# marcobellagente93/scaling

Hardware: AMD Instinct MI355X
Metric: tokens/sec (whole node) Llama-2-7B-shape bf16, TP×PP×DP on 1/2/4/8 MI355X (higher is better)
Workload: dtype bf16

## Files before the change

### csrc/bindings.cpp

```cpp
#include <torch/extension.h>
#include <ATen/hip/HIPContext.h>
#include <c10/core/DeviceGuard.h>

#include <atomic>
#include <cmath>
#include <cstring>
#include <string>
#include <vector>
#include "kernels/launch.h"

void register_rehearsal(pybind11::module& m);
void register_blaslt(pybind11::module& m);

namespace {

hipStream_t cur_stream() { return at::hip::getCurrentHIPStream().stream(); }

int dt(const at::Tensor& t) {
    switch (t.scalar_type()) {
        case at::kFloat: return DT_F32;
        case at::kBFloat16: return DT_BF16;
        case at::kHalf: return DT_F16;
        default: TORCH_CHECK(false, "scaling_amd: unsupported dtype ", t.scalar_type());
    }
// ... 632 lines not shown
        TORCH_CHECK(q.scalar_type() == at::kBFloat16, "flash_attn: FP8 k / v need bfloat16 queries (an e4m3 code times its scale is exact in bfloat16, not in float16)");
        TORCH_CHECK(v.size(0) == k.size(0), "flash_attn: k and v must hold the same number of rows");
        for (const at::Tensor* s : {&*k_scale, &*v_scale})
            TORCH_CHECK(s->is_cuda() && s->scalar_type() == at::kFloat && s->dim() == 2 && s->size(0) == k.size(1) &&
                            s->size(1) == k.size(0) && s->stride(1) == 1 && s->stride(0) == k_scale->stride(0),
                        "flash_attn: k_scale / v_scale must be float32 GPU tensors [kv heads, key rows] with unit last stride");
    } else {
        check_qkv(k, "k"); check_qkv(v, "v");
        TORCH_CHECK(k.scalar_type() == q.scalar_type() && v.scalar_type() == q.scalar_type(), "flash_attn: q/k/v dtypes differ");
    }
    TORCH_CHECK(p_drop >= 0.0 && p_drop < 1.0, "flash_attn: dropout probability must be in [0, 1)");
    const int64_t D = q.size(2);
    TORCH_CHECK(D == 32 || D == 64 || D == 128, "flash_attn: head dim must be 32, 64 or 128");
    TORCH_CHECK(k.size(2) == D && v.size(2) == D && k.size(1) == v.size(1) && q.size(1) % k.size(1) == 0, "flash_attn: shapes");
    TORCH_CHECK(cu_q.scalar_type() == at::kInt && cu_k.scalar_type() == at::kInt && cu_q.numel() == cu_k.numel(), "flash_attn: cu_seqlens int32");
    const at::DeviceGuard g(q.device());
    const int64_t T = q.size(0), H = q.size(1);
    auto o = at::empty({T, H, D}, q.options());
    auto lse = at::empty({H, T}, q.options().dtype(at::kFloat));
    FwdArgs a{};
    a.q = (const uint16_t*)q.data_ptr(); a.k = (const uint16_t*)k.data_ptr(); a.v = (const uint16_t*)v.data_ptr();
    a.o = (uint16_t*)o.data_ptr(); a.lse = lse.data_ptr<float>();
    a.q_tok = q.stride(0); a.q_head = q.stride(1); a.k_tok = k.stride(0); a.k_head = k.stride(1);
    a.v_tok = v.stride(0); a.v_head = v.stride(1); a.o_tok = o.stride(0); a.o_head = o.stride(1); a.lse_stride = T;
    a.cu_q = cu_q.data_ptr<int>(); a.cu_k = cu_k.data_ptr<int>();
    a.nseg = (int)cu_q.numel() - 1; a.Hq = (int)H; a.Hkv = (int)k.size(1); a.causal = causal ? 1 : 0; a.window = (int)window;
    a.local_heads = local_heads < 0 ? (int)H : (int)local_heads;
    a.scale_log2 = (float)(scale * 1.4426950408889634);
    a.p_drop = (float)p_drop; a.rp_drop = (float)(1.0 / (1.0 - p_drop)); a.seed = (uint32_t)seed; a.drop_thr = drop_threshold(p_drop);
    const int64_t grp = H / k.size(1);
    if (k_range.has_value()) {
        TORCH_CHECK(k_range->is_cuda() && k_range->scalar_type() == at::kInt && k_range->is_contiguous() &&
                    k_range->dim() == 2 && k_range->size(0) == a.nseg && k_range->size(1) == 2,
                    "flash_attn: k_range must be a contiguous int32 GPU tensor [nseg, 2]");
        TORCH_CHECK(p_drop == 0.0 && max_q * grp <= 32,
                    "flash_attn: key ranges are supported by the decode kernel only (max_q * heads per kv head <= 32, "
                    "no dropout)");
        TORCH_CHECK(v.size(0) == k.size(0), "flash_attn: k and v must hold the same number of rows");
    }
    if (block_table.has_value()) {
        TORCH_CHECK(k_range.has_value(), "flash_attn: block_table needs k_range (start 0, length per segment)");
        TORCH_CHECK(page_size > 0 && page_size % 32 == 0, "flash_attn: page_size must be a positive multiple of 32");
        TORCH_CHECK(block_table->is_cuda() && block_table->scalar_type() == at::kInt && block_table->dim() == 2 &&
                    block_table->size(0) == a.nseg && block_table->size(1) >= 1 && block_table->stride(1) == 1,
                    "flash_attn: block_table must be an int32 GPU tensor [nseg, max_pages] with unit last stride");
        TORCH_CHECK(k.size(0) > 0 && k.size(0) % page_size == 0 && k.size(0) < (int64_t)1 << 31 &&
                    block_table->size(1) * page_size < (int64_t)1 << 31,
                    "flash_attn: with block_table, k / v must hold a whole number of pages (fewer than 2^31 rows)");
    }
    if (q8)
        TORCH_CHECK(p_drop == 0.0 && max_q * grp <= 32,
                    "flash_attn: FP8 k / v are supported by the decode kernel only (max_q * heads per kv head <= 32, "
                    "no dropout)");
    if (T > 0 && a.nseg > 0 && p_drop == 0.0 && max_q * grp <= 32) {
        DecArgs d{};
        d.q = a.q; d.k = a.k; d.v = a.v;
        d.q_tok = a.q_tok; d.q_head = a.q_head; d.k_tok = a.k_tok; d.k_head = a.k_head; d.v_tok = a.v_tok; d.v_head = a.v_head;
        d.cu_q = a.cu_q; d.cu_k = a.cu_k; d.nseg = a.nseg;
        if (q8) { d.k_scale = k_scale->data_ptr<float>(); d.v_scale = v_scale->data_ptr<float>(); d.s_head = k_scale->stride(0); }
        d.k_range = k_range.has_value() ? k_range->data_ptr<int>() : nullptr; d.k_rows = k.size(0); d.Hq = a.Hq; d.Hkv = a.Hkv; d.causal = a.causal;
        d.window = a.window; d.local_heads = a.local_heads; d.scale_log2 = a.scale_log2; d.Tq = T;
        if (block_table.has_value()) {
            d.block_table = block_table->data_ptr<int>(); d.bt_stride = block_table->stride(0); d.page = (int)page_size;
            d.num_pages = (int)(k.size(0) / page_size); d.max_pages = (int)block_table->size(1);
        }
        sa_launch::fa_decode_plan(max_k > 0 ? max_k : k.size(0), a.Hkv, a.nseg, d.split_keys, d.nsplit);
        auto part_o = at::empty({(int64_t)d.nsplit, T, H, D}, q.options().dtype(at::kFloat));
        auto part_ml = at::empty({(int64_t)d.nsplit, T, H, 2}, q.options().dtype(at::kFloat));
        d.part_o = part_o.data_ptr<float>(); d.part_ml = part_ml.data_ptr<float>();
        d.o = a.o; d.o_tok = a.o_tok; d.o_head = a.o_head; d.lse = a.lse; d.lse_stride = a.lse_stride;
        sa_launch::fa_decode(d, (int)D, q.scalar_type() == at::kHalf, cur_stream());
        return {o, lse};
    }
    if (T > 0 && a.nseg > 0) sa_launch::fa_fwd(a, (int)D, (int)max_q, q.scalar_type() == at::kHalf, cur_stream());
    return {o, lse};
}
std::vector<at::Tensor> fa_bwd(const at::Tensor& dout, const at::Tensor& q, const at::Tensor& k, const at::Tensor& v,
                               const at::Tensor& o, const at::Tensor& lse, const at::Tensor& cu_q, const at::Tensor& cu_k,
                               int64_t max_q, int64_t max_k, double scale, bool causal, int64_t window,
                               const c10::optional<at::Tensor>& dq_out, const c10::optional<at::Tensor>& dk_out,
                               const c10::optional<at::Tensor>& dv_out, double p_drop, int64_t seed, int64_t local_heads,
                               const c10::optional<at::Tensor>& rope_cos, const c10::optional<at::Tensor>& rope_sin,
                               const c10::optional<at::Tensor>& rope_pos, int64_t rope_dim, int64_t rope_seq,
                               bool rope_interleaved) {
    check_qkv(q, "q"); check_qkv(k, "k"); check_qkv(v, "v"); check_qkv(o, "o");
    TORCH_CHECK(k.scalar_type() == q.scalar_type() && v.scalar_type() == q.scalar_type() && o.scalar_type() == q.scalar_type() &&
                dout.scalar_type() == q.scalar_type(), "fa_bwd: dtypes differ");
    auto dO = dout.contiguous();
    check_qkv(dO, "dout");
    const int64_t D = q.size(2), T = q.size(0), H = q.size(1), Tk = k.size(0), Hk = k.size(1);
    const at::DeviceGuard g(q.device());
    auto take = [](const c10::optional<at::Tensor>& t, const at::Tensor& like, const char* n) {
        if (!t.has_value()) return at::empty(like.sizes(), like.options());
        TORCH_CHECK(t->sizes() == like.sizes() && t->scalar_type() == like.scalar_type(), "fa_bwd: ", n, " shape/dtype");
        check_qkv(*t, n);
        return *t;
    };
    auto dq = take(dq_out, q, "dq_out");
    auto dk = take(dk_out, k, "dk_out");
    auto dv = take(dv_out, v, "dv_out");
    auto delta = at::empty({H, T}, q.options().dtype(at::kFloat));
    auto lse2 = at::empty({H, T}, q.options().dtype(at::kFloat));
    BwdArgs a{};
    a.q = (const uint16_t*)q.data_ptr(); a.k = (const uint16_t*)k.data_ptr(); a.v = (const uint16_t*)v.data_ptr();
    a.dO = (const uint16_t*)dO.data_ptr(); a.lse = lse.data_ptr<float>(); a.delta = delta.data_ptr<float>(); a.lse2 = lse2.data_ptr<float>();
    a.dq = (uint16_t*)dq.data_ptr(); a.dk = (uint16_t*)dk.data_ptr(); a.dv = (uint16_t*)dv.data_ptr();
    a.q_tok = q.stride(0); a.q_head = q.stride(1); a.k_tok = k.stride(0); a.k_head = k.stride(1);
    a.v_tok = v.stride(0); a.v_head = v.stride(1); a.do_tok = dO.stride(0); a.do_head = dO.stride(1);
    a.dq_tok = dq.stride(0); a.dq_head = dq.stride(1); a.dk_tok = dk.stride(0); a.dk_head = dk.stride(1);
    a.dv_tok = dv.stride(0); a.dv_head = dv.stride(1); a.lse_stride = T;
    a.cu_q = cu_q.data_ptr<int>(); a.cu_k = cu_k.data_ptr<int>();
    a.nseg = (int)cu_q.numel() - 1; a.Hq = (int)H; a.Hkv = (int)Hk; a.causal = causal ? 1 : 0; a.window = (int)window;
    a.local_heads = local_heads < 0 ? (int)H : (int)local_heads;
    a.scale = (float)scale; a.scale_log2 = (float)(scale * 1.4426950408889634);
    a.p_drop = (float)p_drop; a.rp_drop = (float)(1.0 / (1.0 - p_drop)); a.seed = (uint32_t)seed; a.drop_thr = drop_threshold(p_drop);
    a.hsplit = 1; a.Tk = (int)Tk;
    const int grp = (int)(H / Hk);
    const int64_t kblocks = (max_k + 127) / 128;
    if (causal || window >= 0)
        while (a.hsplit < grp && grp % (2 * a.hsplit) == 0 && Hk * a.hsplit * a.nseg * kblocks < 1024) a.hsplit *= 2;
    at::Tensor part;
    if (a.hsplit > 1) {
        part = at::empty({2, a.hsplit, Tk, Hk, D}, q.options().dtype(at::kFloat));
        a.dk_part = part[0].data_ptr<float>();
        a.dv_part = part[1].data_ptr<float>();
    }
    const bool rope = rope_cos.has_value();
    bool fold = false;
    if (rope) {
        TORCH_CHECK(rope_sin.has_value() && rope_cos->scalar_type() == at::kFloat && rope_sin->scalar_type() == at::kFloat &&
                    rope_cos->is_contiguous() && rope_sin->is_contiguous() && rope_cos->size(-1) == rope_dim / 2 &&
                    (!rope_pos.has_value() ||
                     (rope_pos->scalar_type() == at::kLong && rope_pos->numel() == T && rope_pos->is_contiguous() &&
                      rope_pos->device() == q.device())),
                    "fa_bwd: rope tables / positions (contiguous fp32 tables, contiguous int64 positions of [T])");
        fold = D >= 64 && (rope_interleaved ? rope_dim <= D && rope_dim % 8 == 0 : rope_dim == D) && a.hsplit == 1 &&
               Tk == T;
        if (fold) {
            a.rcos = rope_cos->data_ptr<float>(); a.rsin = rope_sin->data_ptr<float>();
            a.rpos = rope_pos.has_value() ? rope_pos->data_ptr<int64_t>() : nullptr;
            a.rrd = (int)rope_dim; a.rseq = (int)rope_seq; a.ril = rope_interleaved ? 1 : 0;
        }
    }
    if (T > 0 && a.nseg > 0)
        sa_launch::fa_bwd(a, (const uint16_t*)o.data_ptr(), o.stride(0), o.stride(1), T, (int)D, (int)max_q, (int)max_k,
                          q.scalar_type() == at::kHalf, cur_stream());
    if (rope && !fold) {
        const int64_t* pp = rope_pos.has_value() ? rope_pos->data_ptr<int64_t>() : nullptr;
        for (at::Tensor* t : {&dq, &dk}) {
            sa_launch::rope(dt(*t), rope_interleaved, t->data_ptr(), t->stride(0), t->stride(1), t->data_ptr(),
                            t->stride(0), t->stride(1), rope_cos->data_ptr<float>(), rope_sin->data_ptr<float>(), pp,
                            t->size(0), (int)t->size(1), (int)t->size(2), (int)rope_dim, (int)rope_seq, -1.f,
                            cur_stream());
        }
    }
    return {dq, dk, dv};
}
at::Tensor aligned16(const at::Tensor& t) {
    auto c = t.contiguous();
    return (reinterpret_cast<uintptr_t>(c.data_ptr()) % 16 == 0) ? c : c.clone();
}
std::tuple<const void*, int64_t, int64_t, int64_t> mask_view(const c10::optional<at::Tensor>& mask, const at::Tensor& x,
                                                             at::Tensor& keep) {
    if (!mask.has_value()) return {nullptr, 0, 0, 0};
    TORCH_CHECK(mask->scalar_type() == at::kBool, "masked_softmax: mask must be bool");
    auto m = mask->to(x.device()).expand(x.sizes());
    if (m.stride(3) != 1) m = m.contiguous();
    keep = m;
    return {m.data_ptr(), m.stride(0), m.stride(1), m.stride(2)};
}
at::Tensor masked_softmax_fwd(const at::Tensor& x_, const c10::optional<at::Tensor>& mask, double scale, double fill,
                              bool round_scaled) {
    TORCH_CHECK(x_.is_cuda() && x_.dim() == 4, "masked_softmax: x must be a [B, H, Sq, Sk] GPU tensor");
    const at::DeviceGuard g(x_.device());
    auto x = aligned16(x_);
    at::Tensor keep;
    auto [mp, mb, mh, mq] = mask_view(mask, x, keep);
    auto y = at::empty_like(x);
    const int64_t N = x.size(3), rows = x.numel() / std::max<int64_t>(N, 1);
    if (rows > 0 && N > 0)
        sa_launch::masked_softmax_fwd(dt(x), x.data_ptr(), mp, y.data_ptr(), rows, (int)N, (int)x.size(1), (int)x.size(2), mb, mh,
                                      mq, (float)scale, (float)fill, round_scaled, cur_stream());
    return y;
}
at::Tensor masked_softmax_bwd(const at::Tensor& dy_, const at::Tensor& y_, const c10::optional<at::Tensor>& mask, double scale) {
    TORCH_CHECK(y_.is_cuda() && y_.dim() == 4 && dy_.sizes() == y_.sizes() && dy_.scalar_type() == y_.scalar_type(),
                "masked_softmax_bwd: shapes");
    const at::DeviceGuard g(y_.device());
    auto y = aligned16(y_);
    auto dy = aligned16(dy_);
    at::Tensor keep;
    auto [mp, mb, mh, mq] = mask_view(mask, y, keep);
    auto dx = at::empty_like(y);
    const int64_t N = y.size(3), rows = y.numel() / std::max<int64_t>(N, 1);
    if (rows > 0 && N > 0)
        sa_launch::masked_softmax_bwd(dt(y), dy.data_ptr(), y.data_ptr(), mp, dx.data_ptr(), rows, (int)N, (int)y.size(1),
                                      (int)y.size(2), mb, mh, mq, (float)scale, cur_stream());
    return dx;
}
at::Tensor act_fwd(const at::Tensor& x_, int64_t kind) {
    TORCH_CHECK(x_.is_cuda(), "activation: GPU tensor expected");
    const at::DeviceGuard g(x_.device());
    auto x = aligned16(x_);
    auto y = at::empty_like(x);
    if (x.numel() > 0) sa_launch::act_fwd(dt(x), x.data_ptr(), y.data_ptr(), x.numel(), (int)kind, cur_stream());
    return y;
}
at::Tensor act_bwd(const at::Tensor& dy_, const at::Tensor& x_, int64_t kind) {
    TORCH_CHECK(x_.is_cuda() && dy_.sizes() == x_.sizes() && dy_.scalar_type() == x_.scalar_type(), "activation_bwd: shapes");
    const at::DeviceGuard g(x_.device());
    auto x = aligned16(x_);
    auto dy = aligned16(dy_);
    auto dx = at::empty_like(x);
    if (x.numel() > 0) sa_launch::act_bwd(dt(x), dy.data_ptr(), x.data_ptr(), dx.data_ptr(), x.numel(), (int)kind, cur_stream());
    return dx;
}
void spin_us(int64_t us) { sa_launch::spin(us, cur_stream()); }
int64_t gate_flags_alloc(int64_t n) {
    void* p = nullptr;
    const size_t bytes = (size_t)std::max<int64_t>(n, 1) * sizeof(uint32_t);
    TORCH_CHECK(hipHostMalloc(&p, bytes, hipHostMallocCoherent | hipHostMallocMapped) == hipSuccess, "gate: pinned memory");
    std::memset(p, 0, bytes);
    return (int64_t)(uintptr_t)p;
}
void gate_flag_write(int64_t base, int64_t idx, int64_t value) {
    std::atomic_thread_fence(std::memory_order_seq_cst);
    __atomic_store_n(reinterpret_cast<uint32_t*>((uintptr_t)base) + idx, (uint32_t)value, __ATOMIC_SEQ_CST);
}
int64_t gate_flag_read(int64_t base, int64_t idx) {
// ... 64 lines not shown
    m.def("sample_max_resident_vocab", []() { return sa_launch::sample_max_resident(); },
          "the largest vocabulary whose row the sampling kernel stages in LDS");
    m.doc() = "scaling_amd CDNA4 (gfx950) HIP kernels";
    register_rehearsal(m);
    register_blaslt(m);
    m.def("norm_fwd", &norm_fwd, "RMSNorm/LayerNorm forward (optional fused residual add)", py::arg("x"), py::arg("w"), py::arg("b"), py::arg("eps"), py::arg("layer"), py::arg("res") = py::none());
    m.def("norm_bwd", &norm_bwd, "RMSNorm/LayerNorm backward (optional fused residual-gradient add)", py::arg("dy"), py::arg("x"), py::arg("w"), py::arg("mean"), py::arg("rstd"), py::arg("layer"), py::arg("dadd") = py::none());
    m.def("swiglu_fwd", &swiglu_fwd, "SwiGLU forward");
    m.def("swiglu_bwd", &swiglu_bwd, "SwiGLU backward");
    m.def("ar_alloc", &ar_alloc, "one-shot all-reduce: allocate + IPC-export a registered buffer");
    m.def("ar_open", &ar_open, "one-shot all-reduce: map a peer's registered buffer");
    m.def("ar_close", &ar_close, "unmap a peer buffer");
    m.def("ar_free", &ar_free, "free an own registered buffer");
    m.def("ar_allreduce", &ar_allreduce, "one-shot all-reduce of x over the registered buffers (in place)",
          py::arg("x"), py::arg("bases"), py::arg("rank"), py::arg("slot_off"), py::arg("flag_off"), py::arg("epoch"),
          py::arg("signal"), py::arg("err"), py::arg("max_spins") = int64_t(1) << 26);
    m.def("transpose_ok", &transpose_ok, "whether transpose2d supports this tensor");
    m.def("transpose2d", &transpose2d, "x^T (contiguous) for 2-byte 2-D matrices");
    m.def("gemv_ok", &gemv_ok, "whether gemv supports these operands");
    m.def("gemv", &gemv, "y = x W^T (+ b) for at most 4 rows of x (decode-time linear layers)", py::arg("x"), py::arg("W"), py::arg("bias") = py::none());
    m.def("gemv_residual", &gemv_residual, "y = x W^T + res for at most 4 rows (decode MLP-out + residual)");
    m.def("gemv_swiglu", &gemv_swiglu, "y = silu(x Wg^T) * (x Wu^T) for W = [Wg; Wu], at most 4 rows (decode)");
    m.def("gemv_w8_ok", &gemv_w8_ok, "whether the FP8-weight GEMV supports these operands");
    m.def("gemv_w8", &gemv_w8, "y = x (scale * Q)^T (+ b) for at most 4 bf16 rows of x, Q e4m3fn codes, scale fp32 per row",
          py::arg("x"), py::arg("q"), py::arg("scale"), py::arg("bias") = py::none());
    m.def("gemv_w8_residual", &gemv_w8_residual, "gemv_w8 + res (decode down / o-projection + residual)");
    m.def("gemv_w8_swiglu", &gemv_w8_swiglu, "silu(x Wg^T) * (x Wu^T) over FP8 [Wg; Wu] with per-row scales (decode)");
    m.def("gemv_w8_norm_ok", &gemv_w8_norm_ok, "whether gemv_w8_norm supports these operands");
    m.def("gemv_w8_norm", &gemv_w8_norm, "(s, gemv_w8(rms_norm(s), Q, scale)) with s = x (+ add); epi 0 plain, 2 SwiGLU",
          py::arg("x"), py::arg("add"), py::arg("gamma"), py::arg("eps"), py::arg("q"), py::arg("scale"), py::arg("epi") = 0);
    m.def("gemv_norm_ok", &gemv_norm_ok, "whether gemv_norm supports these operands");
    m.def("gemv_norm_rope", &gemv_norm_rope, "graph decode: rms_norm + q/k/v GEMV + interleaved RoPE + K/V cache append "
          "in one launch; returns q or None");
    m.def("gemv_norm", &gemv_norm, "(s, gemv(rms_norm(s), W)) with s = x (+ add); epi 0 plain, 2 SwiGLU (decode)",
          py::arg("x"), py::arg("add"), py::arg("gamma"), py::arg("eps"), py::arg("W"), py::arg("epi") = 0);
    m.def("skinny_ok", &skinny_ok, "whether skinny supports these operands");
    m.def("skinny", &skinny, "y = x W^T (+ b) for at most 16 rows of x on the MFMA weight-streaming kernel (batched decode)",
          py::arg("x"), py::arg("W"), py::arg("bias") = py::none());
    m.def("skinny_residual", &skinny_residual, "y = x W^T + res for at most 16 rows (decode down / o-projection + residual)");
    m.def("skinny_swiglu", &skinny_swiglu, "y = silu(x Wg^T) * (x Wu^T) for W = [Wg; Wu], at most 16 rows (decode)");
    m.def("skinny_norm_ok", &skinny_norm_ok, "whether skinny_norm supports these operands");
    m.def("skinny_norm", &skinny_norm, "(s, skinny(rms_norm(s), W)) with s = x (+ add); epi 0 plain, 2 SwiGLU (decode)",
          py::arg("x"), py::arg("add"), py::arg("gamma"), py::arg("eps"), py::arg("W"), py::arg("epi") = 0);
    m.def("skinny_w8_ok", &skinny_w8_ok, "whether the FP8-weight skinny kernel supports these operands");
    m.def("skinny_w8", &skinny_w8, "y = x (scale * Q)^T (+ b) for at most 16 bf16 rows of x, Q e4m3fn codes, scale fp32 per row",
          py::arg("x"), py::arg("q"), py::arg("scale"), py::arg("bias") = py::none());
    m.def("skinny_w8_residual", &skinny_w8_residual, "skinny_w8 + res (decode down / o-projection + residual)");
    m.def("skinny_w8_swiglu", &skinny_w8_swiglu, "silu(x Wg^T) * (x Wu^T) over FP8 [Wg; Wu] with per-row scales (decode)");
    m.def("skinny_w8_norm_ok", &skinny_w8_norm_ok, "whether skinny_w8_norm supports these operands");
    m.def("skinny_w8_norm", &skinny_w8_norm, "(s, skinny_w8(rms_norm(s), Q, scale)) with s = x (+ add); epi 0 plain, 2 SwiGLU",
          py::arg("x"), py::arg("add"), py::arg("gamma"), py::arg("eps"), py::arg("q"), py::arg("scale"), py::arg("epi") = 0);
    m.def("gemm_tn_ok", &gemm_tn_ok, "whether gemm_tn supports these operands");
    m.def("gemm_tn", &gemm_tn, "C (+)= A^T B for k-major bf16 operands (weight-gradient GEMM)");
    m.def("rope", &rope, "rotary embedding (fwd / inverse), optional strided / in-place output", py::arg("x"), py::arg("cos"), py::arg("sin"), py::arg("pos"), py::arg("rot_dim"), py::arg("seq_len"), py::arg("interleaved"), py::arg("inverse"), py::arg("out") = py::none());
    m.def("rope_kv_append", &rope_kv_append, "graph decode: RoPE q, RoPE k into the K cache row, v into the V cache row (k_scale / v_scale: FP8 e4m3 cache)",
          py::arg("qkv"), py::arg("cos"), py::arg("sin"), py::arg("pos"), py::arg("nq"), py::arg("nkv"), py::arg("rot_dim"), py::arg("interleaved"),
          py::arg("kc"), py::arg("vc"), py::arg("err"), py::arg("k_scale") = py::none(), py::arg("v_scale") = py::none());
    m.def("rope_kv_append_batch", &rope_kv_append_batch, "batched graph decode: rope_kv_append for one token of each of B sequences, one launch",
          py::arg("qkv"), py::arg("cos"), py::arg("sin"), py::arg("pos"), py::arg("nq"), py::arg("nkv"), py::arg("rot_dim"), py::arg("interleaved"),
          py::arg("kc"), py::arg("vc"), py::arg("err"), py::arg("cap"), py::arg("k_scale") = py::none(), py::arg("v_scale") = py::none());
    m.def("rope_kv_append_paged", &rope_kv_append_paged, "paged batched decode: rope_kv_append_batch into the pages a block table names, one launch",
          py::arg("qkv"), py::arg("cos"), py::arg("sin"), py::arg("pos"), py::arg("nq"), py::arg("nkv"), py::arg("rot_dim"), py::arg("interleaved"),
          py::arg("kc"), py::arg("vc"), py::arg("err"), py::arg("block_table"), py::arg("page"), py::arg("k_scale") = py::none(), py::arg("v_scale") = py::none());
    m.def("xent_stats", &xent_stats, "cross-entropy row statistics");
    m.def("xent_bwd", &xent_bwd, "cross-entropy backward");
    m.def("embed_fwd", &embed_fwd, "vocab-parallel embedding forward");
    m.def("embed_bwd", &embed_bwd, "deterministic embedding backward", py::call_guard<py::gil_scoped_release>());
    m.def("adamw_", &adamw_, "fused AdamW on flat fp32 buffers");
    m.def("sumsq_", &sumsq_, "sum of squares + non-finite count");
    m.def("cast_scale_", &cast_scale_, "y = cast(x * scale)");
    m.def("masked_softmax_fwd", &masked_softmax_fwd, "softmax(masked_fill(x * scale, mask, fill)) over the last dim", py::arg("x"), py::arg("mask"), py::arg("scale"), py::arg("fill"), py::arg("round_scaled"));
    m.def("masked_softmax_bwd", &masked_softmax_bwd, "masked softmax backward", py::arg("dy"), py::arg("y"), py::arg("mask"), py::arg("scale"));
    m.def("act_fwd", &act_fwd, "activation forward (0 gelu, 1 silu, 2 gelu-tanh)");
    m.def("act_bwd", &act_bwd, "activation backward");
    m.def("spin_us", &spin_us, "debug: busy-wait kernel of ~us microseconds on the current stream");
    m.def("gate_flags_alloc", &gate_flags_alloc, "stream gates: n flag words (coherent pinned host memory)");
    m.def("gate_flag_write", &gate_flag_write, "stream gates: host store of a flag word (after a full fence)");
    m.def("gate_flag_read", &gate_flag_read, "stream gates: host load of a flag word");
    m.def("gate_stream_wait", &gate_stream_wait, "stream gates: the current stream waits until flag[idx] >= value");
    m.def("xgmi_emulate", &xgmi_emulate, "per-rank proxy: emulated collective (HBM traffic on nwg CUs, held to us)",
          py::arg("src"), py::arg("scratch"), py::arg("bytes"), py::arg("us"), py::arg("nwg") = 16);
    m.def("dropout_add", &dropout_add, "residual + dropout(x) with a hashed keep mask", py::arg("x"), py::arg("res"), py::arg("p"), py::arg("seed"));
    m.def("fa_fwd", &fa_fwd, "flash attention forward (bf16/fp16, optional attention dropout)", py::arg("q"), py::arg("k"), py::arg("v"), py::arg("cu_q"), py::arg("cu_k"), py::arg("max_q"), py::arg("scale"), py::arg("causal"), py::arg("window"), py::arg("p_drop") = 0.0, py::arg("seed") = 0, py::arg("local_heads") = -1, py::arg("max_k") = -1, py::arg("k_range") = py::none(), py::arg("k_scale") = py::none(), py::arg("v_scale") = py::none(), py::arg("block_table") = py::none(), py::arg("page_size") = 0);
    m.def("fa_bwd", &fa_bwd, "flash attention backward (optional strided dq/dk/dv outputs)", py::arg("dout"), py::arg("q"), py::arg("k"), py::arg("v"), py::arg("o"), py::arg("lse"), py::arg("cu_q"), py::arg("cu_k"), py::arg("max_q"), py::arg("max_k"), py::arg("scale"), py::arg("causal"), py::arg("window"), py::arg("dq_out") = py::none(), py::arg("dk_out") = py::none(), py::arg("dv_out") = py::none(), py::arg("p_drop") = 0.0, py::arg("seed") = 0, py::arg("local_heads") = -1, py::arg("rope_cos") = py::none(), py::arg("rope_sin") = py::none(), py::arg("rope_pos") = py::none(), py::arg("rope_dim") = 0, py::arg("rope_seq") = 1, py::arg("rope_interleaved") = false);
}
```

### csrc/kernels/flash_bwd.hip

```cpp
#include "flash_attn.h"
#include "launch.h"

using namespace sa;
using namespace sa::fa;

template <int D, typename E>
__global__ __launch_bounds__(256) void fa_bwd_dot_kernel(const E* __restrict__ o, int64_t o_tok, int64_t o_head,
                                                         const E* __restrict__ dO, int64_t d_tok, int64_t d_head,
                                                         float* __restrict__ delta, const float* __restrict__ lse,
                                                         float* __restrict__ lse2, int64_t T, int H) {
    constexpr int LPR = D / 8;
    const int64_t gid = (int64_t)blockIdx.x * blockDim.x + threadIdx.x;
    const int64_t row = gid / LPR;
    const int c = (int)(gid % LPR);
    float s = 0.f;
    const bool ok = row < T * H;
    int64_t t = 0;
    int hh = 0;
    if (ok) {
        t = row / H;
        hh = (int)(row % H);
        float a[8], b[8];
        V8<E>::ld(o + t * o_tok + hh * o_head + 8 * c, a);
        V8<E>::ld(dO + t * d_tok + hh * d_head + 8 * c, b);
#pragma unroll
        for (int j = 0; j < 8; ++j) s += a[j] * b[j];
    }
#pragma unroll
    for (int w = LPR / 2; w > 0; w >>= 1) s += __shfl_xor(s, w, 64);
    if (ok && c == 0) {
        delta[(int64_t)hh * T + t] = s;
        lse2[(int64_t)hh * T + t] = lse[(int64_t)hh * T + t] * 1.4426950408889634f;
    }
}

template <int D, bool F16>
__device__ __forceinline__ void store_grad_row(const BwdArgs& a, const f32x16 (&acc)[D / 32], float scale, int64_t tok,
                                               int h, u16* dst) {
    constexpr int NT = D / 32;
    auto rd = [&](int t, int g, float (&x)[4]) {
#pragma unroll
        for (int j = 0; j < 4; ++j) x[j] = t2f<F16>(f2t<F16>(acc[t][4 * g + j] * scale));
    };
    auto st = [&](int t, int g, const float (&x)[4]) {
        u16x4 w;
#pragma unroll
        for (int j = 0; j < 4; ++j) w[j] = f2t<F16>(x[j]);
        *reinterpret_cast<u16x4*>(dst + 32 * t + 8 * g + 4 * h) = w;
    };
    if (a.rcos == nullptr) {
#pragma unroll
        for (int t = 0; t < NT; ++t)
#pragma unroll
            for (int g = 0; g < 4; ++g) {
                float x[4];
                rd(t, g, x);
                st(t, g, x);
            }
        return;
    }
    const int64_t ps = a.rpos ? a.rpos[tok] : (tok % a.rseq);
    const float* cb = a.rcos + ps * (a.rrd / 2);
    const float* sb = a.rsin + ps * (a.rrd / 2);
    if constexpr (NT < 2) return;
    if (!a.ril) {
        constexpr int NH = NT / 2 > 0 ? NT / 2 : 1;
        f32x4 cv[NH][4], sv[NH][4];
#pragma unroll
        for (int t = 0; t < NT / 2; ++t)
#pragma unroll
            for (int g = 0; g < 4; ++g) {
                cv[t][g] = *reinterpret_cast<const f32x4*>(cb + 32 * t + 8 * g + 4 * h);
                sv[t][g] = *reinterpret_cast<const f32x4*>(sb + 32 * t + 8 * g + 4 * h);
            }
#pragma unroll
        for (int t = 0; t < NT / 2; ++t)
#pragma unroll
            for (int g = 0; g < 4; ++g) {
                float x[4], y[4];
                rd(t, g, x);
                rd(t + NT / 2, g, y);
#pragma unroll
                for (int j = 0; j < 4; ++j) {
                    float o0, o1;
                    rot_pair(x[j], y[j], cv[t][g][j], -sv[t][g][j], o0, o1);
                    x[j] = o0;
                    y[j] = o1;
                }
                st(t, g, x);
                st(t + NT / 2, g, y);
            }
        return;
    }
    const int hr = a.rrd / 2 - 2;
    float2 cv[NT][4], sv[NT][4];
#pragma unroll
    for (int t = 0; t < NT; ++t)
#pragma unroll
        for (int g = 0; g < 4; ++g) {
            const int p = min((32 * t + 8 * g + 4 * h) / 2, hr);
            cv[t][g] = *reinterpret_cast<const float2*>(cb + p);
            sv[t][g] = *reinterpret_cast<const float2*>(sb + p);
        }
#pragma unroll
    for (int t = 0; t < NT; ++t)
#pragma unroll
        for (int g = 0; g < 4; ++g) {
            const bool rot = 32 * t + 8 * g + 4 * h < a.rrd;
            float x[4];
// ... 182 lines not shown
        if (w + 2 < nwork) {
            issue(ig, iq, buf0);
            adv(ig, iq);
        }
        tile(buf1, cg, cq);
        adv(cg, cq);
        dma_barrier();
    }
    if (w < nwork) tile(buf0, cg, cq);

    if (mykey < Lk) {
        if (a.hsplit > 1) {
            const int64_t pix = (((int64_t)sub * a.Tk + k0s + mykey) * a.Hkv + hk) * D;
            float* kp = a.dk_part + pix;
            float* vp = a.dv_part + pix;
#pragma unroll
            for (int t = 0; t < NT; ++t)
#pragma unroll
                for (int g = 0; g < 4; ++g) {
                    f32x4 wk, wv;
#pragma unroll
                    for (int j = 0; j < 4; ++j) {
                        wk[j] = dk[t][4 * g + j] * a.scale;
                        wv[j] = dv[t][4 * g + j];
                    }
                    *reinterpret_cast<f32x4*>(kp + 32 * t + 8 * g + 4 * h) = wk;
                    *reinterpret_cast<f32x4*>(vp + 32 * t + 8 * g + 4 * h) = wv;
                }
        } else {
            u16* vp = a.dv + (int64_t)(k0s + mykey) * a.dv_tok + (int64_t)hk * a.dv_head;
#pragma unroll
            for (int t = 0; t < NT; ++t)
#pragma unroll
                for (int g = 0; g < 4; ++g) {
                    u16x4 wv;
#pragma unroll
                    for (int j = 0; j < 4; ++j) wv[j] = f2t<F16>(dv[t][4 * g + j]);
                    *reinterpret_cast<u16x4*>(vp + 32 * t + 8 * g + 4 * h) = wv;
                }
            store_grad_row<D, F16>(a, dk, a.scale, k0s + mykey, h,
                                   a.dk + (int64_t)(k0s + mykey) * a.dk_tok + (int64_t)hk * a.dk_head);
        }
    }
#endif
}

template <int D, bool F16, bool DROP>
__global__ __launch_bounds__(256, 2) void fa_bwd_dq_kernel(BwdArgs a) {
#if defined(__HIP_DEVICE_COMPILE__)
    extern __shared__ __attribute__((aligned(16))) char smem[];
    constexpr int TILE = 64 * D * 2, NKS = D / 16, NT = D / 32;
    const int seg = attn_seg(), hq = xcd_head(blockIdx.x, a.Hq);
    const int q0s = a.cu_q[seg], k0s = a.cu_k[seg];
    const int Lq = a.cu_q[seg + 1] - q0s, Lk = a.cu_k[seg + 1] - k0s;
    const int ntiles_q = (Lq + 127) / 128;
    const int qt = attn_qtile(a.causal);
    if (qt >= ntiles_q) return;
    const int hk = hq / (a.Hq / a.Hkv);
    const int win = hq < a.local_heads ? a.window : -1;
    const int tid = threadIdx.x, lane = tid & 63, wave = __builtin_amdgcn_readfirstlane(tid >> 6), h = lane >> 5,
              lq = lane & 31;
    const int wave_u = wave;
    const int off = Lk - Lq;
    const int qwg0 = qt * 128, qw0 = qwg0 + wave * 32, myq = qw0 + lq;
    const int qlast = min(qwg0 + 127, Lq - 1);
    int khi = Lk;
    if (a.causal) khi = min(Lk, qlast + off + 1);
    else if (win >= 0) khi = min(Lk, qlast + off + win + 1);
    int klo = 0;
    if (win >= 0) klo = max(0, qwg0 + off - win);
    klo = (klo / 64) * 64;

    bf16x8 qf[NKS], df[NKS];
    {
        const int qrow = q0s + min(myq, Lq - 1);
        const u16* qp = a.q + (int64_t)qrow * a.q_tok + (int64_t)hq * a.q_head;
        const u16* dp = a.dO + (int64_t)qrow * a.do_tok + (int64_t)hq * a.do_head;
#pragma unroll
        for (int ks = 0; ks < NKS; ++ks) {
            qf[ks] = __builtin_bit_cast(bf16x8, *reinterpret_cast<const u16x8*>(qp + 16 * ks + 8 * h));
            df[ks] = __builtin_bit_cast(bf16x8, *reinterpret_cast<const u16x8*>(dp + 16 * ks + 8 * h));
        }
    }
    const float nl2 = myq < Lq ? -a.lse[(int64_t)hq * a.lse_stride + q0s + myq] * 1.4426950408889634f : -INFINITY;
    const float dlt = myq < Lq ? a.delta[(int64_t)hq * a.lse_stride + q0s + myq] : 0.f;
#pragma unroll
    for (int ks = 0; ks < NKS; ++ks) asm volatile("" ::"v"(qf[ks]), "v"(df[ks]));
    asm volatile("" ::"v"(nl2), "v"(dlt));
    uint32_t drow = 0;
    if constexpr (DROP) drow = drop_row(drop_head(a.seed, hq), q0s + myq);
    LdsOffsets<D> lo;
    lo.init(lane);
    DmaTile<D, 4> tk, tv;
    tk.init(wave_u, lane, a.k_tok);
    tv.init(wave_u, lane, a.v_tok);
    const u16* kbase = a.k + (int64_t)k0s * a.k_tok + (int64_t)hk * a.k_head;
    const u16* vbase = a.v + (int64_t)k0s * a.v_tok + (int64_t)hk * a.v_head;
#define SA_DQ_ISSUE(KT, BUFP)                                                                          \
    do {                                                                                               \
        const int kp_ = (KT);                                                                          \
        dma_load(tk, kbase + (int64_t)kp_ * a.k_tok, a.k_tok, Lk - kp_, (BUFP), wave_u);                 \
        dma_load(tv, vbase + (int64_t)kp_ * a.v_tok, a.v_tok, Lk - kp_, (BUFP) + TILE, wave_u);          \
    } while (0)
    f32x16 dq[NT];
#pragma unroll
    for (int t = 0; t < NT; ++t) dq[t] = f32x16{};
    const float c2 = a.scale_log2;

    auto tile = [&](const char* K, int kt) {
        const char* V = K + TILE;
        const bool need_mask = (kt + 64 > Lk) || (a.causal && kt + 63 > qw0 + off) ||
                               (win >= 0 && (kt < qw0 + 31 + off - win || (!a.causal && kt + 63 > qw0 + off + win)));
#pragma unroll
        for (int b = 0; b < 2; ++b) {
            f32x16 s = f32x16{}, dp = f32x16{};
            {
#pragma unroll
                for (int ks = 0; ks < NKS; ++ks) {
                    s = mma<F16>(rd_row<D>(K, 32 * b * D * 2, lo.row(ks)), qf[ks], s);
                    dp = mma<F16>(rd_row<D>(V, 32 * b * D * 2, lo.row(ks)), df[ks], dp);
                }
            }
#pragma unroll
            for (int r = 0; r < 16; ++r) s[r] = fast_exp2(__builtin_fmaf(s[r], c2, nl2));
            if (need_mask) {
                mask_fence();
                const int base = kt + 32 * b + 4 * h;
                int hi = Lk - 1 - base, low = -1 << 30;
                if (a.causal) hi = min(hi, myq + off - base);
                else if (win >= 0) hi = min(hi, myq + off + win - base);
                if (win >= 0) low = myq + off - win - base;
#pragma unroll
                for (int r = 0; r < 16; ++r) s[r] = (crow(r) <= hi && crow(r) >= low) ? s[r] : 0.f;
            }
#pragma unroll
            for (int r = 0; r < 16; ++r) {
                const float p = s[r];
                if constexpr (DROP) {
                    const bool keep = drop_keep(drow, k0s + kt + 32 * b + 4 * h + crow(r), a.drop_thr);
                    dp[r] = p * ((keep ? dp[r] * a.rp_drop : 0.f) - dlt);
                } else {
                    dp[r] = p * (dp[r] - dlt);
                }
            }
            {
#pragma unroll
                for (int ss = 0; ss < 2; ++ss) {
                    const bf16x8 db = pack_acc_t<F16>(dp, ss);
                    const int kb = (32 * b + 16 * ss) * D * 2;
#pragma unroll
                    for (int t = 0; t < NT; ++t) dq[t] = mma<F16>(rd_tr<D>(K, kb, lo, t), db, dq[t]);
                }
            }
        }
    };

    char* buf0 = smem;
    char* buf1 = smem + 2 * TILE;
    if (klo < khi) SA_DQ_ISSUE(klo, buf0);
    dma_barrier();
    const int ntiles = khi > klo ? (khi - klo + 63) / 64 : 0;
    int kt = klo;
    for (int pr = 0; pr < ntiles / 2; ++pr, kt += 128) {
        SA_DQ_ISSUE(kt + 64, buf1);
        tile(buf0, kt);
        dma_barrier();
        if (kt + 128 < khi) SA_DQ_ISSUE(kt + 128, buf0);
        tile(buf1, kt + 64);
        dma_barrier();
    }
    if (ntiles & 1) tile(buf0, kt);
#undef SA_DQ_ISSUE
    if (myq < Lq)
        store_grad_row<D, F16>(a, dq, a.scale, q0s + myq, h,
                               a.dq + (int64_t)(q0s + myq) * a.dq_tok + (int64_t)hq * a.dq_head);
#endif
}

template <int D, bool F16>
__global__ __launch_bounds__(256) void fa_bwd_reduce_kernel(BwdArgs a) {
    const int64_t gid = (int64_t)blockIdx.x * blockDim.x + threadIdx.x;
    const int64_t per = (int64_t)a.Tk * a.Hkv * (D / 8);
    if (gid >= per) return;
    const int c = (int)(gid % (D / 8));
    const int64_t th = gid / (D / 8);
    const int hk = (int)(th % a.Hkv);
    const int64_t tok = th / a.Hkv;
    const int64_t pstride = (int64_t)a.Tk * a.Hkv * D;
    float sk[8] = {}, sv[8] = {};
    for (int s = 0; s < a.hsplit; ++s) {
        const float* kp = a.dk_part + s * pstride + th * D + 8 * c;
        const float* vp = a.dv_part + s * pstride + th * D + 8 * c;
        float x[8], y[8];
        V8<float>::ld(kp, x);
        V8<float>::ld(vp, y);
#pragma unroll
        for (int j = 0; j < 8; ++j) { sk[j] += x[j]; sv[j] += y[j]; }
    }
    u16x8 wk, wv;
#pragma unroll
    for (int j = 0; j < 8; ++j) { wk[j] = fa::f2t<F16>(sk[j]); wv[j] = fa::f2t<F16>(sv[j]); }
    *reinterpret_cast<u16x8*>(a.dk + tok * a.dk_tok + (int64_t)hk * a.dk_head + 8 * c) = wk;
    *reinterpret_cast<u16x8*>(a.dv + tok * a.dv_tok + (int64_t)hk * a.dv_head + 8 * c) = wv;
}

template <bool F16, bool DROP>
static void launch_bwd_main(const BwdArgs& a, int D, int max_q, int max_k, hipStream_t st) {
    {
        dim3 grid(a.Hkv * a.hsplit, a.nseg, (max_k + 127) / 128);
        const size_t lds = 128 * D * 2 + 2 * (2 * 32 * D * 2 + 512);
        if (D == 128) hipLaunchKernelGGL((fa_bwd_dkdv_kernel<128, F16, DROP>), grid, 256, lds, st, a);
        else if (D == 64) hipLaunchKernelGGL((fa_bwd_dkdv_kernel<64, F16, DROP>), grid, 256, lds, st, a);
        else hipLaunchKernelGGL((fa_bwd_dkdv_kernel<32, F16, DROP>), grid, 256, lds, st, a);
    }
    {
        dim3 grid = attn_grid(a.Hq, a.nseg, (max_q + 127) / 128);
        const size_t lds = 4 * 64 * D * 2;
        if (D == 128) hipLaunchKernelGGL((fa_bwd_dq_kernel<128, F16, DROP>), grid, 256, lds, st, a);
        else if (D == 64) hipLaunchKernelGGL((fa_bwd_dq_kernel<64, F16, DROP>), grid, 256, lds, st, a);
        else hipLaunchKernelGGL((fa_bwd_dq_kernel<32, F16, DROP>), grid, 256, lds, st, a);
    }
    if (a.hsplit > 1) {
        const int64_t threads = (int64_t)a.Tk * a.Hkv * (D / 8);
        const int grid = (int)((threads + 255) / 256);
        if (D == 128) hipLaunchKernelGGL((fa_bwd_reduce_kernel<128, F16>), grid, 256, 0, st, a);
        else if (D == 64) hipLaunchKernelGGL((fa_bwd_reduce_kernel<64, F16>), grid, 256, 0, st, a);
        else hipLaunchKernelGGL((fa_bwd_reduce_kernel<32, F16>), grid, 256, 0, st, a);
    }
}

template <int D, typename T>
static void launch_bwd_dot(const BwdArgs& a, const uint16_t* o, int64_t o_tok, int64_t o_head, int64_t Tq, hipStream_t st) {
    const int64_t threads = Tq * a.Hq * (D / 8);
    const int grid = (int)((threads + 255) / 256);
    hipLaunchKernelGGL((fa_bwd_dot_kernel<D, T>), grid, 256, 0, st, (const T*)o, o_tok, o_head, (const T*)a.dO, a.do_tok,
                       a.do_head, a.delta, a.lse, a.lse2, Tq, a.Hq);
}

template <int D>
static void launch_bwd(const BwdArgs& a, const uint16_t* o, int64_t o_tok, int64_t o_head, int64_t Tq, int max_q,
                       int max_k, bool f16, hipStream_t st) {
    const bool drop = a.p_drop > 0.f;
    if (f16) {
        launch_bwd_dot<D, _Float16>(a, o, o_tok, o_head, Tq, st);
        if (drop) launch_bwd_main<true, true>(a, D, max_q, max_k, st);
        else launch_bwd_main<true, false>(a, D, max_q, max_k, st);
    } else {
        launch_bwd_dot<D, u16>(a, o, o_tok, o_head, Tq, st);
        if (drop) launch_bwd_main<false, true>(a, D, max_q, max_k, st);
        else launch_bwd_main<false, false>(a, D, max_q, max_k, st);
    }
}

namespace sa_launch {
void fa_bwd(const BwdArgs& a, const uint16_t* o, int64_t o_tok, int64_t o_head, int64_t Tq, int D, int max_q, int max_k,
            bool f16, hipStream_t st) {
    if (D == 128) launch_bwd<128>(a, o, o_tok, o_head, Tq, max_q, max_k, f16, st);
    else if (D == 64) launch_bwd<64>(a, o, o_tok, o_head, Tq, max_q, max_k, f16, st);
    else launch_bwd<32>(a, o, o_tok, o_head, Tq, max_q, max_k, f16, st);
}
}
```

### csrc/kernels/launch.h

```cpp
#pragma once
#include <hip/hip_runtime.h>
#include <stdint.h>

enum SaDType { DT_F32 = 0, DT_BF16 = 1, DT_F16 = 2 };

namespace sa_launch {
void norm_fwd(int dtype, bool layer, const void* x, const void* w, const void* b, void* y, float* mean, float* rstd,
              int64_t rows, int H, float eps, hipStream_t st, const void* res = nullptr, void* sum_out = nullptr);
int norm_bwd_waves(int64_t rows, int H);
int64_t norm_bwd_scratch(int64_t rows, int H, bool layer);
void norm_bwd(int dtype, bool layer, const void* dy, const void* x, const void* w, const float* mean,
              const float* rstd, void* dx, void* dw, void* db, float* part, int64_t rows, int H, hipStream_t st,
              const void* dadd = nullptr);
}

struct AppendPages { const int* table; int64_t stride; int page, num_pages; };

namespace sa_launch {
void swiglu_fwd(int dtype, const void* a, const void* b, int64_t lda, void* out, int64_t rows, int F, hipStream_t st);
void swiglu_bwd(int dtype, const void* dy, const void* a, const void* b, int64_t lda, void* da, void* db, int64_t ldd,
                int64_t rows, int F, hipStream_t st);
void rope(int dtype, bool interleaved, const void* x, int64_t x_tok, int64_t x_head, void* out, int64_t o_tok,
          int64_t o_head, const float* cosb, const float* sinb, const int64_t* pos, int64_t T_, int nh, int hd, int rd,
          int seq_len, float sign, hipStream_t st);
bool rope_kv_append(int dtype, bool interleaved, const void* x, void* q_out, void* kc, void* vc, const int64_t* pos,
                    const float* cosb, const float* sinb, int nq, int nkv, int hd, int rd, int64_t lim, int* err,
                    hipStream_t st, int B = 1, int64_t cap = 0, float* k_scale = nullptr, float* v_scale = nullptr,
                    int64_t s_head = 0, const AppendPages* pages = nullptr);
}

namespace sa_launch {
void xent_stats(int dtype, const void* logits, const int64_t* tgt, int64_t rows, int V, int64_t v0, float* m, float* s,
                float* t, int64_t* amax, hipStream_t st);
void xent_bwd(int dtype, const void* logits, const int64_t* tgt, const float* lse, const float* gscale, void* dlogits,
              int64_t rows, int V, int64_t v0, hipStream_t st);
void embed_fwd(int dtype, const int64_t* ids, const void* W, void* out, int64_t ntok, int H, int64_t v0, int64_t Vp,
               hipStream_t st);
void embed_bwd(int dtype, const void* dy, const int64_t* order, const int64_t* sid, int64_t ntok, void* dW, int H,
               int64_t v0, int64_t Vp, hipStream_t st);
void adamw(int gdtype, int pdtype, float* p, const void* g, float* m, float* v, void* pout, int64_t n, float lr,
           float b1, float b2, float eps, float wd, float bc1, float bc2_sqrt, float gscale, hipStream_t st);
int sumsq_blocks(int64_t n);
void sumsq(int dtype, const void* x, int64_t n, float scale, float* part_sq, float* part_bad, float* out_sq,
           float* out_bad, int accumulate, hipStream_t st);
void cast_scale(int sdt, int ddt, const void* x, void* y, int64_t n, float scale, hipStream_t st);
bool transpose_supported(int64_t R, int64_t C, int64_t ld_in);
void transpose_u16(const void* in, int64_t ld_in, void* out, int64_t R, int64_t C, hipStream_t st);
}

namespace sa_launch {
bool gemm_tn_supported(int64_t M, int64_t N, int64_t K, int64_t lda, int64_t ldb, int64_t ldc);
int64_t gemm_tn_plan(int64_t M, int64_t N, int64_t K, int slots, int& full_blocks, int& split);
void gemm_tn(const void* A, int64_t lda, const void* B, int64_t ldb, void* C, int64_t ldc, int64_t M, int64_t N,
             int64_t K, bool beta, hipStream_t st, int full_blocks = -1, int split = 1, float* ws = nullptr);
}

struct FwdArgs {
    const uint16_t* q; const uint16_t* k; const uint16_t* v; uint16_t* o; float* lse;
    int64_t q_tok, q_head, k_tok, k_head, v_tok, v_head, o_tok, o_head, lse_stride;
    const int* cu_q; const int* cu_k;
    int nseg, Hq, Hkv, causal, window;
    int local_heads;
    float scale_log2;
    float p_drop, rp_drop;
    uint32_t seed, drop_thr;
};
namespace sa_launch {
void fa_fwd(const FwdArgs& a, int D, int max_q, bool f16, hipStream_t st);
}

struct DecArgs {
    const uint16_t* q; const uint16_t* k; const uint16_t* v;
    int64_t q_tok, q_head, k_tok, k_head, v_tok, v_head;
    const int* cu_q; const int* cu_k;
    const int* k_range; int64_t k_rows;
    const float* k_scale; const float* v_scale; int64_t s_head;
    int nseg, Hq, Hkv, causal, window, local_heads;
    float scale_log2;
    int split_keys, nsplit;
    int64_t Tq;
    float* part_o;
    float* part_ml;
    uint16_t* o; int64_t o_tok, o_head;
    float* lse; int64_t lse_stride;
    const int* block_table; int64_t bt_stride; int page, num_pages, max_pages;
};
namespace sa_launch {
void fa_decode_plan(int64_t max_k, int Hkv, int nseg, int& split_keys, int& nsplit);
void fa_decode(const DecArgs& a, int D, bool f16, hipStream_t st);
}

struct BwdArgs {
    const uint16_t* q; const uint16_t* k; const uint16_t* v; const uint16_t* dO;
    const float* lse; float* delta; float* lse2;
    uint16_t* dq; uint16_t* dk; uint16_t* dv;
    int64_t q_tok, q_head, k_tok, k_head, v_tok, v_head, do_tok, do_head;
    int64_t dq_tok, dq_head, dk_tok, dk_head, dv_tok, dv_head, lse_stride;
    const int* cu_q; const int* cu_k;
    int nseg, Hq, Hkv, causal, window;
    int local_heads;
    float scale, scale_log2;
    float p_drop, rp_drop;
    uint32_t seed, drop_thr;
    int hsplit, Tk;
    float* dk_part;
    float* dv_part;
    const float* rcos; const float* rsin; const int64_t* rpos;
    int rrd, rseq, ril;
};
namespace sa_launch {
void fa_bwd(const BwdArgs& a, const uint16_t* o, int64_t o_tok, int64_t o_head, int64_t Tq, int D, int max_q, int max_k,
            bool f16, hipStream_t st);
}

namespace sa_launch {
void masked_softmax_fwd(int dtype, const void* x, const void* mask, void* y, int64_t rows, int N, int H, int Sq, int64_t mb,
                        int64_t mh, int64_t mq, float scale, float fill, bool round, hipStream_t st);
void masked_softmax_bwd(int dtype, const void* dy, const void* y, const void* mask, void* dx, int64_t rows, int N, int H,
                        int Sq, int64_t mb, int64_t mh, int64_t mq, float scale, hipStream_t st);
void act_fwd(int dtype, const void* x, void* y, int64_t n, int kind, hipStream_t st);
void act_bwd(int dtype, const void* dy, const void* x, void* dx, int64_t n, int kind, hipStream_t st);
void dropout(int dtype, const void* x, const void* res, void* out, int64_t n, uint32_t seed, uint32_t thr, float rp,
             hipStream_t st);
}

namespace sa_launch {
void spin(int64_t us, hipStream_t st);
void xgmi_emulate(const void* src, int64_t src_bytes, void* scratch, int64_t scratch_bytes, int64_t bytes, double us,
                  int nwg, hipStream_t st);
void oneshot_allreduce(int dtype, char* const* bases, int world, int rank, int64_t slot_off, int64_t flag_off,
                       uint32_t epoch, bool signal, void* out, int64_t n, int* err, int64_t max_spins,
                       hipStream_t st);
}

namespace sa_launch {
int sample_max_resident();
void sample(int dtype, const void* logits, int64_t ld, int64_t B, int V, int64_t* tokens, int* info,
            const int64_t* step, uint32_t seed, int top_k, float top_p, float temperature, hipStream_t st);
}

struct GemvRope {
    const float* cosb; const float* sinb; const int64_t* pos;
    void* q_out; void* kc; void* vc;
    int nq, nkv, hd, rd;
    int64_t lim; int* err;
};
namespace sa_launch {
void gemv(int dtype, int M, const void* x, int64_t ldx, const void* W, int64_t ldw, const float* scale, const void* b,
          void* y, int64_t ldy, int N, int K, hipStream_t st, int epi = 0, const void* res = nullptr, int64_t ldr = 0,
          const void* norm_w = nullptr, const void* norm_add = nullptr, void* norm_sum = nullptr, float eps = 0.f,
          const struct GemvRope* rope = nullptr);
void skinny(int dtype, int M, const void* x, int64_t ldx, const void* W, int64_t ldw, const float* scale, const void* b,
            void* y, int64_t ldy, int N, int K, hipStream_t st, int epi = 0, const void* res = nullptr, int64_t ldr = 0,
            const void* norm_w = nullptr, const void* norm_add = nullptr, void* norm_sum = nullptr, float eps = 0.f);
}
```

Baseline: 32850.

## Fold flash-attention backward delta computation into the dq kernel and run it first

Flash-attention backward no longer runs a separate dot kernel for delta = rowsum(O·dO). The dq kernel now computes delta itself from O and dO and writes delta and lse2 to global memory. The dq kernel is launched before the dkdv kernel so that kernel can read those values. This removes one kernel launch and one extra pass over O/dO, but reorders the kernels and adds O loads and a reduction to the dq kernel.

```diff
diff --git a/csrc/bindings.cpp b/csrc/bindings.cpp
--- a/csrc/bindings.cpp
+++ b/csrc/bindings.cpp
@@ -738,7 +738,7 @@
                                const c10::optional<at::Tensor>& dv_out, double p_drop, int64_t seed, int64_t local_heads,
                                const c10::optional<at::Tensor>& rope_cos, const c10::optional<at::Tensor>& rope_sin,
                                const c10::optional<at::Tensor>& rope_pos, int64_t rope_dim, int64_t rope_seq,
-                               bool rope_interleaved) {
+                               bool rope_interleaved, bool fold_delta) {
     check_qkv(q, "q"); check_qkv(k, "k"); check_qkv(v, "v"); check_qkv(o, "o");
     TORCH_CHECK(k.scalar_type() == q.scalar_type() && v.scalar_type() == q.scalar_type() && o.scalar_type() == q.scalar_type() &&
                 dout.scalar_type() == q.scalar_type(), "fa_bwd: dtypes differ");
@@ -759,6 +759,7 @@
     auto lse2 = at::empty({H, T}, q.options().dtype(at::kFloat));
     BwdArgs a{};
     a.q = (const uint16_t*)q.data_ptr(); a.k = (const uint16_t*)k.data_ptr(); a.v = (const uint16_t*)v.data_ptr();
+    a.o = (const uint16_t*)o.data_ptr(); a.o_tok = o.stride(0); a.o_head = o.stride(1); a.fold_delta = fold_delta ? 1 : 0;
     a.dO = (const uint16_t*)dO.data_ptr(); a.lse = lse.data_ptr<float>(); a.delta = delta.data_ptr<float>(); a.lse2 = lse2.data_ptr<float>();
     a.dq = (uint16_t*)dq.data_ptr(); a.dk = (uint16_t*)dk.data_ptr(); a.dv = (uint16_t*)dv.data_ptr();
     a.q_tok = q.stride(0); a.q_head = q.stride(1); a.k_tok = k.stride(0); a.k_head = k.stride(1);
@@ -799,8 +800,7 @@
         }
     }
     if (T > 0 && a.nseg > 0)
-        sa_launch::fa_bwd(a, (const uint16_t*)o.data_ptr(), o.stride(0), o.stride(1), T, (int)D, (int)max_q, (int)max_k,
-                          q.scalar_type() == at::kHalf, cur_stream());
+        sa_launch::fa_bwd(a, T, (int)D, (int)max_q, (int)max_k, q.scalar_type() == at::kHalf, cur_stream());
     if (rope && !fold) {
         const int64_t* pp = rope_pos.has_value() ? rope_pos->data_ptr<int64_t>() : nullptr;
         for (at::Tensor* t : {&dq, &dk}) {
@@ -1031,5 +1031,5 @@
           py::arg("src"), py::arg("scratch"), py::arg("bytes"), py::arg("us"), py::arg("nwg") = 16);
     m.def("dropout_add", &dropout_add, "residual + dropout(x) with a hashed keep mask", py::arg("x"), py::arg("res"), py::arg("p"), py::arg("seed"));
     m.def("fa_fwd", &fa_fwd, "flash attention forward (bf16/fp16, optional attention dropout)", py::arg("q"), py::arg("k"), py::arg("v"), py::arg("cu_q"), py::arg("cu_k"), py::arg("max_q"), py::arg("scale"), py::arg("causal"), py::arg("window"), py::arg("p_drop") = 0.0, py::arg("seed") = 0, py::arg("local_heads") = -1, py::arg("max_k") = -1, py::arg("k_range") = py::none(), py::arg("k_scale") = py::none(), py::arg("v_scale") = py::none(), py::arg("block_table") = py::none(), py::arg("page_size") = 0);
-    m.def("fa_bwd", &fa_bwd, "flash attention backward (optional strided dq/dk/dv outputs)", py::arg("dout"), py::arg("q"), py::arg("k"), py::arg("v"), py::arg("o"), py::arg("lse"), py::arg("cu_q"), py::arg("cu_k"), py::arg("max_q"), py::arg("max_k"), py::arg("scale"), py::arg("causal"), py::arg("window"), py::arg("dq_out") = py::none(), py::arg("dk_out") = py::none(), py::arg("dv_out") = py::none(), py::arg("p_drop") = 0.0, py::arg("seed") = 0, py::arg("local_heads") = -1, py::arg("rope_cos") = py::none(), py::arg("rope_sin") = py::none(), py::arg("rope_pos") = py::none(), py::arg("rope_dim") = 0, py::arg("rope_seq") = 1, py::arg("rope_interleaved") = false);
-}
+    m.def("fa_bwd", &fa_bwd, "flash attention backward (optional strided dq/dk/dv outputs)", py::arg("dout"), py::arg("q"), py::arg("k"), py::arg("v"), py::arg("o"), py::arg("lse"), py::arg("cu_q"), py::arg("cu_k"), py::arg("max_q"), py::arg("max_k"), py::arg("scale"), py::arg("causal"), py::arg("window"), py::arg("dq_out") = py::none(), py::arg("dk_out") = py::none(), py::arg("dv_out") = py::none(), py::arg("p_drop") = 0.0, py::arg("seed") = 0, py::arg("local_heads") = -1, py::arg("rope_cos") = py::none(), py::arg("rope_sin") = py::none(), py::arg("rope_pos") = py::none(), py::arg("rope_dim") = 0, py::arg("rope_seq") = 1, py::arg("rope_interleaved") = false, py::arg("fold_delta") = true);
+}
diff --git a/csrc/kernels/flash_bwd.hip b/csrc/kernels/flash_bwd.hip
--- a/csrc/kernels/flash_bwd.hip
+++ b/csrc/kernels/flash_bwd.hip
@@ -24,7 +24,7 @@
         V8<E>::ld(o + t * o_tok + hh * o_head + 8 * c, a);
         V8<E>::ld(dO + t * d_tok + hh * d_head + 8 * c, b);
 #pragma unroll
-        for (int j = 0; j < 8; ++j) s += a[j] * b[j];
+        for (int j = 0; j < 8; ++j) s = __builtin_fmaf(a[j], b[j], s);
     }
 #pragma unroll
     for (int w = LPR / 2; w > 0; w >>= 1) s += __shfl_xor(s, w, 64);
@@ -373,8 +373,39 @@
             df[ks] = __builtin_bit_cast(bf16x8, *reinterpret_cast<const u16x8*>(dp + 16 * ks + 8 * h));
         }
     }
-    const float nl2 = myq < Lq ? -a.lse[(int64_t)hq * a.lse_stride + q0s + myq] * 1.4426950408889634f : -INFINITY;
-    const float dlt = myq < Lq ? a.delta[(int64_t)hq * a.lse_stride + q0s + myq] : 0.f;
+    const int64_t sx = (int64_t)hq * a.lse_stride + q0s + myq;
+    const float l2 = myq < Lq ? a.lse[sx] * 1.4426950408889634f : INFINITY;
+    const float nl2 = -l2;
+    float dlt = 0.f;
+    if (a.fold_delta) {
+        const u16* op = a.o + (int64_t)(q0s + min(myq, Lq - 1)) * a.o_tok + (int64_t)hq * a.o_head;
+        u16x8 of[NKS];
+#pragma unroll
+        for (int ks = 0; ks < NKS; ++ks) of[ks] = *reinterpret_cast<const u16x8*>(op + 16 * ks + 8 * h);
+        float part[NKS];
+#pragma unroll
+        for (int ks = 0; ks < NKS; ++ks) {
+            const u16x8 dr = __builtin_bit_cast(u16x8, df[ks]);
+            float s = 0.f;
+#pragma unroll
+            for (int j = 0; j < 8; ++j) s = __builtin_fmaf(t2f<F16>(of[ks][j]), t2f<F16>(dr[j]), s);
+            part[ks] = s;
+        }
+#pragma unroll
+        for (int w = NKS / 2; w > 0; w >>= 1)
+#pragma unroll
+            for (int ks = 0; ks < w; ++ks) part[ks] += part[ks + w];
+        const float dsum = sum_xchg32(part[0]);
+        if (myq < Lq) {
+            dlt = dsum;
+            if (h == 0) {
+                a.delta[sx] = dsum;
+                a.lse2[sx] = l2;
+            }
+        }
+    } else if (myq < Lq) {
+        dlt = a.delta[sx];
+    }
 #pragma unroll
     for (int ks = 0; ks < NKS; ++ks) asm volatile("" ::"v"(qf[ks]), "v"(df[ks]));
     asm volatile("" ::"v"(nl2), "v"(dlt));
@@ -496,7 +527,17 @@
 }
 
 template <bool F16, bool DROP>
+static void launch_bwd_dq(const BwdArgs& a, int D, int max_q, hipStream_t st) {
+    dim3 grid = attn_grid(a.Hq, a.nseg, (max_q + 127) / 128);
+    const size_t lds = 4 * 64 * D * 2;
+    if (D == 128) hipLaunchKernelGGL((fa_bwd_dq_kernel<128, F16, DROP>), grid, 256, lds, st, a);
+    else if (D == 64) hipLaunchKernelGGL((fa_bwd_dq_kernel<64, F16, DROP>), grid, 256, lds, st, a);
+    else hipLaunchKernelGGL((fa_bwd_dq_kernel<32, F16, DROP>), grid, 256, lds, st, a);
+}
+
+template <bool F16, bool DROP>
 static void launch_bwd_main(const BwdArgs& a, int D, int max_q, int max_k, hipStream_t st) {
+    if (a.fold_delta) launch_bwd_dq<F16, DROP>(a, D, max_q, st);
     {
         dim3 grid(a.Hkv * a.hsplit, a.nseg, (max_k + 127) / 128);
         const size_t lds = 128 * D * 2 + 2 * (2 * 32 * D * 2 + 512);
@@ -504,13 +545,7 @@
         else if (D == 64) hipLaunchKernelGGL((fa_bwd_dkdv_kernel<64, F16, DROP>), grid, 256, lds, st, a);
         else hipLaunchKernelGGL((fa_bwd_dkdv_kernel<32, F16, DROP>), grid, 256, lds, st, a);
     }
-    {
-        dim3 grid = attn_grid(a.Hq, a.nseg, (max_q + 127) / 128);
-        const size_t lds = 4 * 64 * D * 2;
-        if (D == 128) hipLaunchKernelGGL((fa_bwd_dq_kernel<128, F16, DROP>), grid, 256, lds, st, a);
-        else if (D == 64) hipLaunchKernelGGL((fa_bwd_dq_kernel<64, F16, DROP>), grid, 256, lds, st, a);
-        else hipLaunchKernelGGL((fa_bwd_dq_kernel<32, F16, DROP>), grid, 256, lds, st, a);
-    }
+    if (!a.fold_delta) launch_bwd_dq<F16, DROP>(a, D, max_q, st);
     if (a.hsplit > 1) {
         const int64_t threads = (int64_t)a.Tk * a.Hkv * (D / 8);
         const int grid = (int)((threads + 255) / 256);
@@ -521,33 +556,31 @@
 }
 
 template <int D, typename T>
-static void launch_bwd_dot(const BwdArgs& a, const uint16_t* o, int64_t o_tok, int64_t o_head, int64_t Tq, hipStream_t st) {
+static void launch_bwd_dot(const BwdArgs& a, int64_t Tq, hipStream_t st) {
     const int64_t threads = Tq * a.Hq * (D / 8);
     const int grid = (int)((threads + 255) / 256);
-    hipLaunchKernelGGL((fa_bwd_dot_kernel<D, T>), grid, 256, 0, st, (const T*)o, o_tok, o_head, (const T*)a.dO, a.do_tok,
-                       a.do_head, a.delta, a.lse, a.lse2, Tq, a.Hq);
+    hipLaunchKernelGGL((fa_bwd_dot_kernel<D, T>), grid, 256, 0, st, (const T*)a.o, a.o_tok, a.o_head, (const T*)a.dO,
+                       a.do_tok, a.do_head, a.delta, a.lse, a.lse2, Tq, a.Hq);
 }
 
 template <int D>
-static void launch_bwd(const BwdArgs& a, const uint16_t* o, int64_t o_tok, int64_t o_head, int64_t Tq, int max_q,
-                       int max_k, bool f16, hipStream_t st) {
+static void launch_bwd(const BwdArgs& a, int64_t Tq, int max_q, int max_k, bool f16, hipStream_t st) {
     const bool drop = a.p_drop > 0.f;
     if (f16) {
-        launch_bwd_dot<D, _Float16>(a, o, o_tok, o_head, Tq, st);
+        if (!a.fold_delta) launch_bwd_dot<D, _Float16>(a, Tq, st);
         if (drop) launch_bwd_main<true, true>(a, D, max_q, max_k, st);
         else launch_bwd_main<true, false>(a, D, max_q, max_k, st);
     } else {
-        launch_bwd_dot<D, u16>(a, o, o_tok, o_head, Tq, st);
+        if (!a.fold_delta) launch_bwd_dot<D, u16>(a, Tq, st);
         if (drop) launch_bwd_main<false, true>(a, D, max_q, max_k, st);
         else launch_bwd_main<false, false>(a, D, max_q, max_k, st);
     }
 }
 
 namespace sa_launch {
-void fa_bwd(const BwdArgs& a, const uint16_t* o, int64_t o_tok, int64_t o_head, int64_t Tq, int D, int max_q, int max_k,
-            bool f16, hipStream_t st) {
-    if (D == 128) launch_bwd<128>(a, o, o_tok, o_head, Tq, max_q, max_k, f16, st);
-    else if (D == 64) launch_bwd<64>(a, o, o_tok, o_head, Tq, max_q, max_k, f16, st);
-    else launch_bwd<32>(a, o, o_tok, o_head, Tq, max_q, max_k, f16, st);
-}
-}
+void fa_bwd(const BwdArgs& a, int64_t Tq, int D, int max_q, int max_k, bool f16, hipStream_t st) {
+    if (D == 128) launch_bwd<128>(a, Tq, max_q, max_k, f16, st);
+    else if (D == 64) launch_bwd<64>(a, Tq, max_q, max_k, f16, st);
+    else launch_bwd<32>(a, Tq, max_q, max_k, f16, st);
+}
+}
diff --git a/csrc/kernels/launch.h b/csrc/kernels/launch.h
--- a/csrc/kernels/launch.h
+++ b/csrc/kernels/launch.h
@@ -92,6 +92,7 @@
 
 struct BwdArgs {
     const uint16_t* q; const uint16_t* k; const uint16_t* v; const uint16_t* dO;
+    const uint16_t* o; int64_t o_tok, o_head; int fold_delta;
     const float* lse; float* delta; float* lse2;
     uint16_t* dq; uint16_t* dk; uint16_t* dv;
     int64_t q_tok, q_head, k_tok, k_head, v_tok, v_head, do_tok, do_head;
@@ -109,8 +110,7 @@
     int rrd, rseq, ril;
 };
 namespace sa_launch {
-void fa_bwd(const BwdArgs& a, const uint16_t* o, int64_t o_tok, int64_t o_head, int64_t Tq, int D, int max_q, int max_k,
-            bool f16, hipStream_t st);
+void fa_bwd(const BwdArgs& a, int64_t Tq, int D, int max_q, int max_k, bool f16, hipStream_t st);
 }
 
 namespace sa_launch {
```

Result: no change. 32980, median of 6 (+0.4%).
